# lpastura/kubernetes-1

Measured on AMD Instinct MI355X. Metric: pods scheduled/sec, higher is better.
Workload: dtype int64; 1 GPU; (b) 5000 nodes / 1913000 pods; nodes=5000, nodes_per_gpu=5000, pods=1913000, percentage_of_nodes_to_score=100, parallelism=1 GPU

## Files before the change

include/kgpu.h:

```cpp
#ifndef KGPU_H
#define KGPU_H

#include <stdint.h>

#ifdef __cplusplus
extern "C" {
#endif

#define KGPU_ABI_VERSION 3

#define KGPU_OK 0
#define KGPU_E_INVAL (-1)
#define KGPU_E_NOMEM (-2)
#define KGPU_E_DEVICE (-3)
#define KGPU_E_CAPACITY (-4)
#define KGPU_E_STATE (-5)
#define KGPU_E_UNSUPPORTED (-6)

#define KGPU_CODE_SUCCESS 0
#define KGPU_CODE_ERROR 1
#define KGPU_CODE_UNSCHEDULABLE 2
#define KGPU_CODE_UNRESOLVABLE 3

#define KGPU_F_NODE_UNSCHEDULABLE 0
// ... 392 lines not shown
#define KGPU_OPT_BATCH_GEO 11
#define KGPU_OPT_ARENA_BYTES 12
#define KGPU_OPT_TOPO_RESIDENT 13
#define KGPU_OPT_BATCH_HELPER 14
#define KGPU_OPT_TOPO_AHEAD 15
#define KGPU_OPT_TBATCH_GEO 16
#define KGPU_OPT_HOLD_GROUP 17
#define KGPU_OPT_TBATCH_WLAB 18
#define KGPU_OPT_RUN_ALL_FILTERS 20
#define KGPU_OPT_TBATCH_POLL_SLEEP 21
#define KGPU_OPT_ZEROCOPY_POOLS 23
#define KGPU_OPT_CUT_PERSISTENT 24
#define KGPU_OPT_CUT_TOPO_PERSISTENT 25
#define KGPU_OPT_NORM_PERSISTENT 26
#define KGPU_OPT_BATCH_EARLY_PUBLISH 27
int kgpu_set_option(kgpu_ctx* ctx, int32_t option, int64_t value);
int kgpu_debug_counters(const kgpu_ctx* ctx, int64_t* out, int32_t n);
int kgpu_geometry_for(int32_t kernel, int32_t n_nodes, int32_t max_groups, int32_t first, int32_t out[4]);
int kgpu_debug_geometry(const kgpu_ctx* ctx, int32_t out[6]);
int kgpu_debug_instantiation(const kgpu_ctx* ctx, int32_t out[4]);
int kgpu_debug_topo_resident(const kgpu_ctx* ctx, int64_t out[2]);
int kgpu_read_phase_trace(kgpu_ctx* ctx, int64_t* out, int32_t max_iters);

typedef struct kgpu_nominated {
  int32_t node;
  int32_t item;
} kgpu_nominated;
int kgpu_set_nominated(kgpu_ctx* ctx, const kgpu_nominated* noms, int32_t n, const kgpu_pod_query* pods,
                       const kgpu_pools* pools);

// ... 64 lines not shown
```

kubernetes-1_amd/csrc/kgpu_api.cpp:

```cpp
#include <hip/hip_runtime.h>
#include <rccl/rccl.h>
#include <dlfcn.h>
#include <execinfo.h>
#include <fcntl.h>
#include <signal.h>
#include <unistd.h>

#include <algorithm>
#include <array>
#include <chrono>
#include <atomic>
#include <exception>
#include <memory>
#include <new>
#include <iterator>
#include <cmath>
#include <cstdio>
#include <cstdlib>
#include <cstddef>
#include <cstring>
#include <deque>
#include <map>
#include <string>
#include <unordered_map>
// ... 149 lines not shown
    std::string key;
    DevBuf buf[2];
    size_t dirty[2] = {0, 0};
    int cur = 0;
  } tc;
  uint64_t tc_hits = 0, tc_misses = 0;
  bool htrace = false;
  static constexpr int kHt = 18;
  int64_t ht_last = 0, ht_cur[kHt] = {}, ht_n = 0;
  int ht_seen = 0;
  std::vector<std::array<int64_t, kHt>> ht_cycles;
  std::vector<std::array<int64_t, kHt>> ht_batches;
  bool tc_on = true;
  bool batch_helper = true;
  bool batch_early = true;
  bool topo_ahead = true;
  int tbatch_geo_first = 1;
  size_t ar_limit = 1 << 20;
  DevState ds_last{};
  const void* ds_ptr = nullptr;
  bool last_diag = false;
  std::vector<int64_t> trace_wg_host;
  int32_t trace_wg_groups = 0;
  std::vector<hipEvent_t> ev_pool;
  std::map<std::vector<int64_t>, int> class_ids, tclass_ids;
  std::vector<kgpu::ClassRec> classes;
  std::vector<kgpu::ClassItem> citems;
  std::vector<kgpu::TermClassRec> tclasses;
  std::vector<kgpu_req> creqs;
  std::vector<int32_t> cints;
// ... 109 lines not shown
      c->err = std::string(msg) + (what.empty() ? "" : ": " + what) +
               (invalidate ? " (device mirror invalidated: upload the snapshot again)" : "");
    } catch (...) {
      c->err.clear();
    }
  }
  return code;
}

void note_geometry(kgpu_ctx* c, int kernel, int geo, int groups, int per) {
  int threads = 0, rows = 0;
  kgpu::geometry_shape(kernel, geo, &threads, &rows);
  const int32_t v[6] = {kernel, geo, threads, rows, groups, per};
  std::copy(v, v + 6, c->last_geo);
}
void note_instantiation(kgpu_ctx* c, int row, bool xg, bool helper, int pods) {
  c->last_inst[0] = row;
  c->last_inst[1] = xg ? 1 : 0;
  c->last_inst[2] = helper ? 1 : 0;
  c->last_inst[3] += pods;
}
void reset_geometry(kgpu_ctx* c) {
  const int32_t v[6] = {0, -1, 0, 0, 0, 0};
  std::copy(v, v + 6, c->last_geo);
  const int32_t w[4] = {-1, 0, 0, 0};
  std::copy(w, w + 4, c->last_inst);
}

#define HIP_OK(c, x)                                                                           \
  do {                                                                                         \
    hipError_t e_ = (x);                                                                       \
    if (e_ != hipSuccess)                                                                      \
      return fail((c), KGPU_E_DEVICE, std::string(#x ": ") + hipGetErrorString(e_));           \
  } while (0)

// ... 1967 lines not shown
        ba.GT = groups;
      } else if (xg) {
        const size_t cells = (size_t)kgpu::kXgmiRing * (size_t)c->xg_GT;
        ba.gran = static_cast<uint64_t*>(c->xg_box.p);
        ba.feas = reinterpret_cast<int32_t*>(ba.gran + cells);
        ba.pgran = static_cast<uint64_t* const*>(c->xg_arr.p);
        ba.pfeas = reinterpret_cast<int32_t* const*>(static_cast<uint64_t* const*>(c->xg_arr.p) + c->xg_nranks);
        ba.nranks = c->xg_nranks;
        ba.rank = c->xg_rank;
        ba.GT = c->xg_GT;
        ba.R = kgpu::kXgmiRing;
        ba.xseq0 = c->xg_seq;
        c->xg_seq += cnt;
      } else {
        ba.dual = c->batch_early && kgpu::batch_helper_used(c->spec, kidx, false, c->batch_helper) ? 1 : 0;
        const size_t cells = (size_t)cnt * (size_t)groups * (ba.dual ? 2 : 1);
        const size_t gbytes = sizeof(uint64_t) * cells + sizeof(int32_t) * cells;
        if ((rc = ensure(c, c->gran, gbytes))) return rc;
        HIP_OK(c, hipMemsetAsync(c->gran.p, 0, sizeof(uint64_t) * cells, c->stream));
        ba.gran = static_cast<uint64_t*>(c->gran.p);
        ba.feas = reinterpret_cast<int32_t*>(ba.gran + cells);
        run_ptrs.push_back({ba.gran, ba.feas});
        void** slot = static_cast<void**>(c->batch_ptrs.p) + 2 * (run_ptrs.size() - 1);
        if ((rc = stage_h2d(c, slot, run_ptrs.back().data(), sizeof(void*) * 2))) return rc;
        ba.pgran = reinterpret_cast<uint64_t* const*>(slot);
        ba.pfeas = reinterpret_cast<int32_t* const*>(slot + 1);
        ba.nranks = 1;
        ba.rank = 0;
        ba.GT = groups;
        ba.R = 0;
      }
      ba.first = i;
      ba.count = cnt;
      ba.per = per;
      ba.assume = assume;
      ba.seq0 = first_seq + i;
      ba.abort = abort_word;
      ba.abort_at = c->abort_at >= i && c->abort_at < i + cnt ? c->abort_at - i : -1;
      ba.skip_release_at = c->skip_release_at >= i && c->skip_release_at < i + cnt ? c->skip_release_at - i : -1;
      ba.trace = nullptr;
      if (c->phase_trace) {
        if ((rc = ensure(c, c->trace, sizeof(int64_t) * 16 * (size_t)(cnt + 1)))) return rc;
        HIP_OK(c, hipMemsetAsync(c->trace.p, 0, sizeof(int64_t) * 16 * (size_t)(cnt + 1), c->stream));
        ba.trace = static_cast<int64_t*>(c->trace.p);
        c->trace_host.assign((size_t)(cnt + 1) * 16, 0);
      }
      if (c->timing) HIP_OK(c, hipEventRecord(get_event(c, ev), c->stream));
      const bool coop = c->coop || c->force_coop;
      ba.hold = coop ? -1 : c->hold_group;
      ++c->n_persist;
      c->n_coop += coop ? 1 : 0;
      ++c->state_launches;
      note_geometry(c, 1, kidx, groups, per);
      note_instantiation(c, kgpu::batch_row(c->spec), ba.R > 0,
                         !cut && kgpu::batch_helper_used(c->spec, kidx, ba.R > 0, c->batch_helper), cnt);
      if (cut) {
        c->n_cut_pods += cnt;
        cut_pods += cnt;
        if (kgpu::launch_cbatch(dst, ba, groups, kidx, c->spec, coop, c->stream))
          return fail(c, KGPU_E_DEVICE, "k_cbatch launch failed");
      } else if (kgpu::launch_batch(dst, ba, groups, kidx, c->spec, coop, c->batch_helper, c->stream))
        return fail(c, KGPU_E_DEVICE, "k_batch launch failed");
      if (c->timing) HIP_OK(c, hipEventRecord(get_event(c, ev + 1), c->stream));
      ev += 2;
      timed_passes += cnt;
      if (ba.trace)
        HIP_OK(c, hipMemcpyAsync(c->trace_host.data(), ba.trace, sizeof(int64_t) * 16 * (size_t)(cnt + 1),
                                 hipMemcpyDeviceToHost, c->stream));
      used_persistent = true;
    } else {
      while (j < n && (kidx < 0 || norm[(size_t)j]) && !topo[(size_t)j] && (nrm.empty() || !nrm[(size_t)j])) ++j;
      int prev = -1;
      bool resolved_in_final = false;
      for (int32_t k = i; k < j; ++k) {
        PodArgs a{};
        a.pod = k;
        a.prev = prev;
        a.prev_blocks = blocks;
        a.prev_parity = (k - 1) & 1;
        a.parity = k & 1;
        const bool one_launch = short_cycle && n == 1 && diag && !sharded && !cut &&
                                !(qs[k].flags & KGPU_Q_SCORE_ERROR) && !needs_norm(c, qs[k], pools);
// ... 850 lines not shown
  void* ptrs[2] = {gran, feas};
  std::memcpy(h + p_off, ptrs, sizeof(ptrs));
  std::memset(h + a_off, 0, 64);
  HIP_OK(c, hipMemcpyAsync(d, h, bytes, hipMemcpyHostToDevice, c->stream));
  c->tc.valid = false;
  kgpu::BatchArgs ba{};
  ba.gran = gran;
  ba.feas = feas;
  ba.pgran = reinterpret_cast<uint64_t* const*>(d + p_off);
  ba.pfeas = reinterpret_cast<int32_t* const*>(d + p_off + sizeof(void*));
  ba.nranks = 1;
  ba.rank = 0;
  ba.GT = groups;
  ba.R = 0;
  ba.dual = dual ? 1 : 0;
  ba.first = 0;
  ba.count = n;
  ba.per = per;
  ba.assume = 1;
  ba.seq0 = first_seq;
  ba.abort = reinterpret_cast<int32_t*>(d + a_off);
  ba.abort_at = -1;
  ba.skip_release_at = -1;
  ba.trace = nullptr;
  ba.res_out = static_cast<kgpu_result*>(ps.res_dev);
  ba.abort_out = reinterpret_cast<int32_t*>(static_cast<char*>(ps.res_dev) + sizeof(kgpu_result) * (size_t)n);
  kgpu_ctx::PipeSlot& po = c->pipe[s ^ 1];
  ba.zero_buf = static_cast<uint64_t*>(po.gran.p);
  ba.zero_n16 = po.gran.p ? (int64_t)(po.gran.bytes / 16) : 0;
  const bool coop = c->coop;
  ba.hold = -1;
  ++c->n_persist;
  c->n_coop += coop ? 1 : 0;
  *reinterpret_cast<int32_t*>(static_cast<char*>(ps.res) + sizeof(kgpu_result) * (size_t)n) = -1;
  const bool timed = stats != nullptr;
  if (timed) HIP_OK(c, hipEventRecord(ps.t0, c->stream));
  note_geometry(c, 1, kidx, groups, per);
  note_instantiation(c, kgpu::batch_row(c->spec), false, kgpu::batch_helper_used(c->spec, kidx, false, c->batch_helper), n);
  if (kgpu::launch_batch(reinterpret_cast<const DevState*>(d), ba, groups, kidx, c->spec, coop, c->batch_helper,
                         c->stream))
    return fail(c, KGPU_E_DEVICE, "k_batch launch failed");
  if (timed) HIP_OK(c, hipEventRecord(ps.t1, c->stream));
  HIP_OK(c, hipEventRecord(ps.done, c->stream));
  ps.gran_zeroed = 0;
  if (po.gran.p) po.gran_zeroed = po.gran.bytes;
  kgpu_ctx::PipeBatch b;
  b.slot = s;
  b.n = n;
  b.results = results;
  b.stats = stats;
  b.timed = timed;
  b.qs.assign(qs, qs + n);
  if (pools) {
// ... 166 lines not shown
  fail_point();
  std::unique_ptr<kgpu_ctx> holder(new kgpu_ctx());
  kgpu_ctx* c = holder.get();
  int ndev = 0;
  if (hipGetDeviceCount(&ndev) != hipSuccess || ndev <= 0) return KGPU_E_DEVICE;
  if (cfg->device < 0 || cfg->device >= ndev) return KGPU_E_INVAL;
  c->cfg = *cfg;
  c->device = cfg->device;
  if (hipSetDevice(c->device) != hipSuccess) return KGPU_E_DEVICE;
  {
    const char* e = std::getenv("KGPU_SYNC_SPIN");
    if (e && e[0] == '1') (void)hipSetDeviceFlags(hipDeviceScheduleSpin);
  }
  if (const char* e = std::getenv("KGPU_HOST_TRACE")) c->htrace = e[0] == '1';
  if (const char* e = std::getenv("KGPU_BATCH_EARLY_PUBLISH")) c->batch_early = e[0] != '0';
  if (hipStreamCreateWithFlags(&c->stream, hipStreamNonBlocking) != hipSuccess)
    return KGPU_E_DEVICE;
  hipDeviceProp_t prop;
  if (hipGetDeviceProperties(&prop, c->device) != hipSuccess) {
    (void)hipStreamDestroy(c->stream);
    return KGPU_E_DEVICE;
  }
  c->n_cus = prop.multiProcessorCount;
  DevState& st = c->st;
  st.n_filters = cfg->n_filters;
  std::memcpy(st.filters, cfg->filters, sizeof(st.filters));
  st.n_scores = cfg->n_scores;
  std::memcpy(st.scores, cfg->scores, sizeof(st.scores));
  for (int i = 0; i < KGPU_NUM_SCORES; ++i) st.weights[i] = std::max<int64_t>(cfg->score_weights[i], 1);
  for (int i = 0; i < KGPU_NUM_SCORES; ++i) st.w_of[i] = 0;
// ... 200 lines not shown
    return fail(c, KGPU_E_STATE, "pipelined batches in flight: complete them with kgpu_schedule_batch_wait first");
  if (!c) return KGPU_E_INVAL;
  if (option == KGPU_OPT_KERNEL_TIMING) c->timing = value != 0;
  else if (option == KGPU_OPT_PERSISTENT) c->persistent = value != 0;
  else if (option == KGPU_OPT_PERSIST_GROUPS) c->max_groups = (int)std::max<int64_t>(value, 0);
  else if (option == KGPU_OPT_PHASE_TRACE) {
    c->phase_trace = value != 0;
    c->phase_trace_mode = (int)std::min<int64_t>(std::max<int64_t>(value, 0), 3);
  }
  else if (option == KGPU_OPT_TOPO_FUSED) c->topo_fused = value != 0;
  else if (option == KGPU_OPT_TOPO_PERSISTENT) c->tfast = value != 0;
  else if (option == KGPU_OPT_COOPERATIVE) c->coop = value != 0;
  else if (option == KGPU_OPT_BATCH_GEO) c->batch_geo_first = (int)std::min<int64_t>(std::max<int64_t>(0, value), 6);
  else if (option == KGPU_OPT_BATCH_HELPER) c->batch_helper = value != 0;
  else if (option == KGPU_OPT_BATCH_EARLY_PUBLISH) c->batch_early = value != 0;
  else if (option == KGPU_OPT_TOPO_AHEAD) c->topo_ahead = value != 0;
  else if (option == KGPU_OPT_TBATCH_GEO) c->tbatch_geo_first = (int)std::min<int64_t>(std::max<int64_t>(value, 0), 4);
  else if (option == KGPU_OPT_TOPO_RESIDENT) {
    c->tc_on = value != 0;
    c->tc.valid = false;
  } else if (option == KGPU_OPT_ARENA_BYTES) c->ar_limit = (size_t)std::min<int64_t>(std::max<int64_t>(0, value), (int64_t)kArenaBytes);
  else if (option == KGPU_OPT_ABORT_AT) c->abort_at = value < 0 || value > INT32_MAX ? -1 : (int32_t)value;
  else if (option == KGPU_OPT_XGMI) c->xgmi = value != 0;
  else if (option == KGPU_OPT_TBATCH_WLAB) c->tbatch_wlab = value != 0;
  else if (option == KGPU_OPT_TBATCH_POLL_SLEEP) c->tbatch_sleep = value != 0;
  else if (option == KGPU_OPT_ZEROCOPY_POOLS) c->zc_pools = value != 0;
  else if (option == KGPU_OPT_RUN_ALL_FILTERS) c->run_all = value != 0;
  else if (option == KGPU_OPT_HOLD_GROUP) c->hold_group = value < 0 || value > INT32_MAX ? -1 : (int32_t)value;
  else if (option == KGPU_OPT_CUT_PERSISTENT) c->cut_persistent = value != 0;
  else if (option == KGPU_OPT_CUT_TOPO_PERSISTENT) c->cut_topo_persistent = value != 0;
// ... 1063 lines not shown
```

kubernetes-1_amd/csrc/kgpu_internal.h:

```cpp
#pragma once
#include <stdint.h>

#include "../../include/kgpu.h"

namespace kgpu {

constexpr int kBlock = 64;
constexpr int kMaxBlocks = 1024;
constexpr int kSelAnd = 0, kSelNothing = 1, kSelEmpty = 2;
constexpr uint64_t kMask40 = (1ull << 40) - 1;
constexpr int kMaxRanks = 64;

struct BlkStat {
  int32_t feasible;
  int32_t max_taint;
  int32_t max_na;
  int32_t pad;
};
struct BlkKey {
  uint64_t key;
  int32_t idx;
  int32_t feasible;
};

// ... 195 lines not shown
  int32_t hold;
  int32_t dual;
  kgpu_result* res_out;
  int32_t* abort_out;
  uint64_t* zero_buf;
  int64_t zero_n16;
  uint64_t* const* pgran;
  int32_t* const* pfeas;
  int32_t nranks, rank;
  int32_t GT;
  int32_t R;
  int64_t xseq0;
  uint64_t* cgran;
  uint64_t* cpos;
  int32_t cut_nofilt;
  int32_t pad_c;
};
constexpr int32_t kAbortDirty = 1, kAbortClean = 2;
constexpr int kXgmiRing = 4096;
constexpr int kXgmiMaxGT = 1024;

constexpr int kTMaxSoftWords = 8;
constexpr int kTMaxZones = 32;
constexpr int kTLdsBudget = 144 * 1024;
constexpr int kTCutBytes = 544;

struct THist {
  int32_t col_kind;
  int32_t col;
  int32_t key;
  int32_t sig;
// ... 160 lines not shown
int launch_vict_prep(const DevState* st, const PreemptArgs* a, void* stream);
int launch_victims(const DevState* st, const PreemptArgs* a, int N, void* stream);

int launch_eval(const DevState* st, const PodArgs& a, int blocks, int spec, void* stream);
int select_spec(const int32_t* filters, int nf, const int32_t* scores, int ns, bool def_res);
int launch_final(const DevState* st, const PodArgs& a, int blocks, int stat_blocks, void* stream);
int launch_cut(const DevState* st, const PodArgs& a, int blocks, int n_filters, void* stream);
int launch_resolve(const DevState* st, int N, const PodArgs& a, void* stream);
int eval_blocks(int N);
int launch_shard_pack(const DevState* st, int parity, int blocks, int what, void* stream);
int batch_geometry(int N, int max_groups, int* per, int* groups, int first = 0);
bool geometry_shape(int kernel, int geo, int* threads, int* rows);
int launch_batch(const DevState* st, const BatchArgs& a, int groups, int kidx, int spec, bool coop, bool helper,
                 void* stream);
int batch_row(int spec);
int launch_cbatch(const DevState* st, const BatchArgs& a, int groups, int kidx, int spec, bool coop, void* stream);
bool batch_helper_used(int spec, int geo, bool sharded, bool helper);
int launch_nbatch(const DevState* st, const BatchArgs& a, int groups, int kidx, int spec, bool coop, void* stream);
constexpr int kNormTaintBits = 20;
bool nbatch_row_ok(int spec);
int launch_topo(const DevState* st, PodArgs a, int blocks, int64_t min_values, int64_t next_scratch,
                bool fused, unsigned long long* bar, unsigned long long bar_base, int n_filters, void* stream,
                const PreemptArgs* nom = nullptr, int N = 0);
inline int topo_barriers(int64_t min_values) { return min_values > 0 ? 5 : 4; }
int launch_class_init(const DevState* st, int c0, int nc, int n_pods, void* stream);
int launch_debug_broken_linear(const kgpu_shape_point* pts, int n_pts, const int64_t* p, int64_t* out, int n,
                               void* stream);
int launch_debug_arith(int op, const int64_t* a, const int64_t* b, const int64_t* c, const int64_t* d, int64_t* out,
                       int32_t* flag, int n, void* stream);
int launch_topo_phase(const DevState* st, const PodArgs& a, int phase, int blocks, int64_t extra, void* stream);
// ... 45 lines not shown
```

kubernetes-1_amd/csrc/kgpu_kernels.hip:

```cpp
#include <hip/hip_runtime.h>

#include <algorithm>
#include <map>
#include <mutex>
#include <tuple>
#include <type_traits>

#include "kgpu_internal.h"

#if defined(__HIP_DEVICE_COMPILE__)
#define GAS __attribute__((address_space(1)))
#define CAS __attribute__((address_space(4)))
#else
#define GAS
#define CAS
#endif

namespace kgpu {

template <class T>
__device__ __forceinline__ GAS T* gp(T* p) {
  return (GAS T*)p;
}
template <class T>
__device__ __forceinline__ const CAS T* cp(const T* p) {
  return (const CAS T*)p;
}


constexpr uint32_t kRuntime = 0xFFFFFFFFu;
// ... 1165 lines not shown
    __builtin_amdgcn_s_sleep(1);
    if ((it & 63) == 0) {
      const uint64_t now = __builtin_amdgcn_s_memrealtime();
      if (it == 0) {
        t0 = now;
      } else if (now - t0 > 2 * kSpinTimeout) {
        __hip_atomic_fetch_or(abort_word, kAbortDirty, __ATOMIC_RELAXED, __HIP_MEMORY_SCOPE_AGENT);
        return;
      }
    }
  }
}
__device__ __forceinline__ void lds_wait(int* f, int v, int32_t* abort_word) { lds_wait_t<false>(f, v, abort_word); }
__device__ __forceinline__ void lds_wait_ge(int* f, int v, int32_t* abort_word) { lds_wait_t<true>(f, v, abort_word); }

__device__ __forceinline__ constexpr bool spare_slot(int j, int K, int tid, int B) {
  return j == K - 1 && tid == B - 1;
}

template <int K, int B>
__device__ __forceinline__ void wg_partials(BatchShared<B>& sh, int p, const uint64_t (&keys)[K], bool vb, int ob,
                                            int jb, int cand, Cand& ra, Cand& rb) {
  const int tid = threadIdx.x, lane = tid & 63, wave = tid >> 6;
  Cand a{0, -1, 0}, b{0, -1, 0};
  if (!vb) {
#pragma unroll
    for (int j = 0; j < K; ++j) {
      const uint64_t k = spare_slot(j, K, tid, B) ? 0 : keys[j];
      a.feas += __popcll(__ballot(k != 0));
      if (k > a.key) { a.key = k; a.idx = j * B + tid; }
// ... 198 lines not shown
  q.nz[0] = s.nz[0]; q.nz[1] = s.nz[1];
  q.score_req[0] = s.score_req[0]; q.score_req[1] = s.score_req[1];
  q.scalars = s.scalars;
  q.ports = s.ports;
  return q;
}
__device__ __forceinline__ kgpu_pod_query ring_uniform(kgpu_pod_query q) {
  q.flags = __builtin_amdgcn_readfirstlane(q.flags);
  q.scalars.begin = __builtin_amdgcn_readfirstlane(q.scalars.begin);
  q.scalars.count = __builtin_amdgcn_readfirstlane(q.scalars.count);
  q.ports.begin = __builtin_amdgcn_readfirstlane(q.ports.begin);
  q.ports.count = __builtin_amdgcn_readfirstlane(q.ports.count);
  return q;
}

template <uint32_t FM, uint32_t SM, int K, int B, bool XG, bool HB = false, bool TR = false, bool EP = false>
__global__ __launch_bounds__(B + 64 + (HB ? 2 * B : 0)) void k_batch(const DevState* __restrict__ stp, BatchArgs pa) {
  static_assert(!HB || (B == 64 && !XG &&
                       SM == ((1u << KGPU_S_BALANCED_ALLOCATION) | (1u << KGPU_S_LEAST_ALLOCATED) | kDefRes)),
                "the helper wave splits config (b)'s profile on the one-row-wave geometry");
  static_assert(HB || !TR, "only the helper-wave instantiation has a traced twin");
  static_assert(HB || !EP, "only the helper-wave instantiation publishes early");
  const DevState& st = *stp;
  constexpr int W = B / 64;
  const int tid = threadIdx.x, wave = tid >> 6, lane = tid & 63;
  const int G = gridDim.x, g = blockIdx.x;
  if (g == pa.hold) return;
  const int lo = g * pa.per;
  const int GT = pa.GT, gme = pa.rank * G + g;
  constexpr bool xg = XG;
  const uint64_t tmask = xg ? (0xFull << 60) : kGValid;
  __shared__ BatchShared<B> sh;
  __shared__ int64_t sh_hk[HB ? 2 * 2 * K * B : 1];
  __shared__ int sh_hready[2];
  __shared__ std::conditional_t<HB, kgpu_pod_query, NoQuery> sh_q[HB ? kQRing : 1];
  __shared__ uint64_t* sh_peer_g[XG ? kMaxRanks : 1];
  __shared__ int32_t* sh_peer_f[XG ? kMaxRanks : 1];
  if constexpr (XG) {
    if (wave == W && lane < pa.nranks) {
      sh_peer_g[lane] = pa.pgran[lane];
      sh_peer_f[lane] = pa.pfeas[lane];
    }
  }
  if (tid == 0) {
    sh.bready = 0;
    sh.cready = 0;
    sh_hready[0] = 0;
    sh_hready[1] = 0;
  }
  if constexpr (HB) {
    if (wave == W && lane < kQWords)
      for (int k = 0; k < 3 && k < pa.count; ++k)
        reinterpret_cast<qword_t*>(&sh_q[k])[lane] = ((const GAS qword_t*)(st.queries + pa.first + k))[lane];
  }
  __syncthreads();
  auto ring_row = [&](int k) -> size_t { return xg ? (size_t)((pa.xseq0 + k) % pa.R) : (size_t)k; };
  auto ring_tag = [&](int k) -> uint64_t {
    return xg ? (kGValid | ((uint64_t)(((pa.xseq0 + k) / pa.R) & 7) << 60)) : kGValid;
  };
  auto publish = [&](int i, uint64_t key, int feas) {
    const size_t roff = ring_row(i) * GT + gme;
    const uint64_t gtag = ring_tag(i);
    if constexpr (!XG) {
// ... 8 lines not shown
  };
  auto publish2 = [&](int i, uint64_t ka, uint64_t kb, int fa, int fb) {
    const size_t roff = (size_t)i * GT + gme;
    typedef uint32_t __attribute__((ext_vector_type(4))) u32x4;
    const uint64_t wa = kGValid | ka, wb = kGValid | kb;
    const u32x4 v = {(uint32_t)wa, (uint32_t)(wa >> 32), (uint32_t)wb, (uint32_t)(wb >> 32)};
    GAS uint64_t* gp2 = (GAS uint64_t*)(pa.gran + 2 * roff);
    asm volatile("global_store_dwordx4 %0, %1, off sc1\n\ts_nop 1" ::"v"(gp2), "v"(v) : "memory");
    reinterpret_cast<int2*>(pa.feas)[roff] = int2{fa, fb};
  };
  const bool tr = pa.trace && (g == 0 || g == G - 1);
  int64_t* trow = pa.trace ? pa.trace + (g == 0 ? 0 : 8) : nullptr;
  constexpr bool kStamps = !HB || TR;
#define KGPU_STAMP(i, k) \
  if (kStamps && tr && (tid == 0 || tid == B)) trow[(size_t)(i) * 16 + (k)] = (int64_t)__builtin_amdgcn_s_memrealtime()

  if constexpr (HB) {
    if (wave == W + 1 || wave == W + 2) {
      const int hw = wave - W - 1;
      HRow h[K];
#pragma unroll
      for (int j = 0; j < K; ++j) {
        const int n = lo + j * B + lane;
        h[j] = HRow{0, 0, 0, 0, 0.0, 0.0};
        if (!spare_slot(j, K, lane, B) && n < st.N) {
          h[j].ac = gp(st.alloc_cpu)[n];
          h[j].am = gp(st.alloc_mem)[n];
          h[j].zc = gp(st.nz_cpu)[n];
          h[j].zm = gp(st.nz_mem)[n];
          h[j].ic = (h[j].ac > 0 && h[j].ac < (1ll << 52)) ? 1.0 / (double)h[j].ac : 0.0;
// ... 24 lines not shown
                t.zm = lane64(h[j].zm, ob) + rqp.nz[1];
                t.ic = __builtin_bit_cast(double, lane64(__builtin_bit_cast(int64_t, h[j].ic), ob));
                t.im = __builtin_bit_cast(double, lane64(__builtin_bit_cast(int64_t, h[j].im), ob));
              }
            if (lane == B - 1) h[K - 1] = t;
          }
          kgpu_pod_query qh;
          qh.score_req[0] = rq.score_req[0];
          qh.score_req[1] = rq.score_req[1];
#pragma unroll
          for (int j = 0; j < K; ++j) {
            const bool spare = spare_slot(j, K, lane, B);
            const int n = spare ? lo + cand : lo + j * B + lane;
            NodeRes nr{};
            nr.ac = h[j].ac; nr.am = h[j].am; nr.zc = h[j].zc; nr.zm = h[j].zm; nr.ic = h[j].ic; nr.im = h[j].im;
            sh_hk[((hw * 2 + p) * K + j) * B + lane] =
                hw == 0 ? least_score<true>(st, qh, nr, n) * wl : balanced_score(qh, nr) * wbal;
          }
          if (lane == 0) lds_release(&sh_hready[hw], i + 1);
        }
        __syncthreads();
        int wg = -1;
        if (have_prev) {
          if (sh.rabort[(i - 1) & 1]) break;
          wg = sh.rwg[(i - 1) & 1];
        }
        const bool won = have_prev && wg == gme;
        if (won && pa.assume && lane == ob) {
#pragma unroll
          for (int j = 0; j < K; ++j)
            if (j == jb) {
              h[j].zc += rqp.nz[0];
              h[j].zm += rqp.nz[1];
            }
// ... 153 lines not shown
        }
        assume_regs(qp, t);
        if (tid == B - 1) r[KR - 1] = t;
      }
      if constexpr (HB) {
        uint32_t fs[K];
        uint64_t rkj[K];
#pragma unroll
        for (int j = 0; j < K; ++j) {
          const bool spare = spare_slot(j, K, tid, B);
          const int n = spare ? lo + cand : lo + j * B + tid;
          fs[j] = (spare ? fast_b : n < st.N) ? run_filters<FM>(st, q, r[j], n) : 1u;
          rkj[j] = rank40(tk, (uint64_t)(st.node_base + n), st.tie_mode);
        }
        if (q.scalars.count | q.ports.count) vm_drain();
        lds_wait_ge(&sh_hready[0], i + 1, pa.abort);
        lds_wait_ge(&sh_hready[1], i + 1, pa.abort);
#pragma unroll
        for (int j = 0; j < K; ++j) {
          const int64_t tot = sh_hk[((0 * 2 + p) * K + j) * B + tid] + sh_hk[((1 * 2 + p) * K + j) * B + tid];
          keys[j] = fs[j] ? 0 : (((uint64_t)(tot + 1) << 40) | rkj[j]);
        }
      } else {
#pragma unroll
        for (int j = 0; j < K; ++j) {
          const bool spare = spare_slot(j, K, tid, B);
          const int n = spare ? lo + cand : lo + j * B + tid;
          if constexpr (kStream) {
            const bool live = spare ? fast_b : n < st.N;
            NodeRes rj = r[0];
            if (!spare && live) rj = load_row<kRecip>(st, n);
            keys[j] = live ? node_key<FM, SM>(st, q, rj, n, tk) : 0;
          } else {
            keys[j] = (spare ? fast_b : n < st.N) ? node_key<FM, SM>(st, q, r[j], n, tk) : 0;
          }
        }
// ... 83 lines not shown
#pragma unroll
        for (int j = 0; j < K; ++j)
          if (j == cand / B) {
            if constexpr (kStream) sh.brow[p] = load_row<kRecip>(st, lo + cand);
            else sh.brow[p] = r[j];
          }
        if (i != pa.skip_release_at) lds_release(&sh.bready, i + 1);
      }
    }
    staged = have_cur && !slow && cand >= 0;
    qp = q;
    q = qn;
    KGPU_STAMP(i, 4);
  }
#undef KGPU_STAMP
}

__global__ __launch_bounds__(256) void k_batch_fixup(const DevState* __restrict__ stp, BatchArgs pa, int G) {
  const DevState& st = *stp;
  const int lane = threadIdx.x & 63;
  const int i = blockIdx.x * 4 + (threadIdx.x >> 6);
  for (int64_t z = (int64_t)blockIdx.x * blockDim.x + threadIdx.x; z < pa.zero_n16; z += (int64_t)gridDim.x * blockDim.x) {
    uint4* zp = reinterpret_cast<uint4*>(pa.zero_buf) + z;
    *zp = uint4{0, 0, 0, 0};
  }
  if (pa.abort_out && blockIdx.x == 0 && threadIdx.x == 0)
    __hip_atomic_store(pa.abort_out, load_sc1(pa.abort), __ATOMIC_RELAXED, __HIP_MEMORY_SCOPE_SYSTEM);
  if (i >= pa.count) return;
  const size_t row = pa.R > 0 ? (size_t)((pa.xseq0 + i) % pa.R) : (size_t)i;
  int f = 0;
// ... 2772 lines not shown
template <uint32_t FM, uint32_t SM>
struct BatchRow {
  using Fn = void (*)(const DevState*, BatchArgs);
  static constexpr Fn fn[kNumGeo] = {k_batch<FM, SM, 1, 64, false>,  k_batch<FM, SM, 1, 128, false>,
                                     k_batch<FM, SM, 1, 192, false>, k_batch<FM, SM, 1, 448, false>,
                                     k_batch<FM, SM, 1, 960, false>, k_batch<FM, SM, 4, 512, false>,
                                     k_batch<FM, SM, 8, 512, false>};
  static constexpr Fn xfn[kNumGeo] = {k_batch<FM, SM, 1, 64, true>,  k_batch<FM, SM, 1, 128, true>,
                                      k_batch<FM, SM, 1, 192, true>, k_batch<FM, SM, 1, 448, true>,
                                      k_batch<FM, SM, 1, 960, true>, k_batch<FM, SM, 4, 512, true>,
                                      k_batch<FM, SM, 8, 512, true>};
};
using BatchFn = void (*)(const DevState*, BatchArgs);
template <uint32_t FM, uint32_t SM, bool E>
struct HelperFn {
  static constexpr BatchFn fn = nullptr, traced = nullptr, early = nullptr, early_traced = nullptr;
};
template <uint32_t FM, uint32_t SM>
struct HelperFn<FM, SM, true> {
  static constexpr BatchFn fn = k_batch<FM, SM, 1, 64, false, true>;
  static constexpr BatchFn traced = k_batch<FM, SM, 1, 64, false, true, true>;
  static constexpr BatchFn early = k_batch<FM, SM, 1, 64, false, true, false, true>;
  static constexpr BatchFn early_traced = k_batch<FM, SM, 1, 64, false, true, true, true>;
};
static const BatchFn kBatchHelper[] = {
    nullptr,
    HelperFn<kFitFM, kFitSM, true>::fn,
    nullptr,
    nullptr,
};
static const BatchFn kBatchHelperTraced[] = {
    nullptr,
    HelperFn<kFitFM, kFitSM, true>::traced,
    nullptr,
    nullptr,
};
static const BatchFn kBatchHelperEarly[] = {
    nullptr,
    HelperFn<kFitFM, kFitSM, true>::early,
    nullptr,
    nullptr,
};
static const BatchFn kBatchHelperEarlyTraced[] = {
    nullptr,
    HelperFn<kFitFM, kFitSM, true>::early_traced,
    nullptr,
    nullptr,
};
static const BatchFn* const kBatch[] = {
    BatchRow<kRuntime, kRuntime>::fn,
    BatchRow<kFitFM, kFitSM>::fn,
    BatchRow<kDefaultFM, kDefaultSM>::fn,
    BatchRow<kDefaultFM, kAutoscalerSM>::fn,
};
static_assert(sizeof(kBatch) / sizeof(kBatch[0]) == kNumSpecs, "one k_batch row per profile instantiation");
static const BatchFn* const kBatchX[] = {
    BatchRow<kRuntime, kRuntime>::xfn,
    BatchRow<kFitFM, kFitSM>::xfn,
    BatchRow<kDefaultFM, kDefaultSM>::xfn,
    BatchRow<kDefaultFM, kAutoscalerSM>::xfn,
};

int batch_geometry(int N, int max_groups, int* per, int* groups, int first) {
// ... 26 lines not shown
int batch_row(int spec) { return spec < 0 || spec >= kNumSpecs ? 0 : spec; }

bool batch_helper_used(int spec, int geo, bool sharded, bool helper) {
  return helper && !sharded && geo == 0 && kBatchHelper[batch_row(spec)] != nullptr;
}

int launch_batch(const DevState* st, const BatchArgs& a, int groups, int geo, int spec, bool coop, bool helper,
                 void* stream) {
  spec = batch_row(spec);
  if (geo < 0 || geo >= kNumGeo) return -1;
  const int x = a.R > 0 ? 1 : 0;
  const bool hb = batch_helper_used(spec, geo, x != 0, helper);
  const bool traced = hb && a.trace != nullptr;
  const bool early = a.dual != 0;
  if (early && !hb) return -1;
  const BatchFn fn = hb ? (early ? (traced ? kBatchHelperEarlyTraced : kBatchHelperEarly)
                                 : (traced ? kBatchHelperTraced : kBatchHelper))[spec]
                        : (x ? kBatchX : kBatch)[spec][geo];
  const int threads = kGeo[geo].B + 64 + (hb ? 2 * kGeo[geo].B : 0);
  static bool attr_set[6][kNumSpecs][kNumGeo] = {};
  const int ai = hb ? (traced ? 3 : 2) + (early ? 2 : 0) : x;
  if (!attr_set[ai][spec][geo]) {
    if (hipFuncSetAttribute(reinterpret_cast<const void*>(fn), hipFuncAttributeMaxDynamicSharedMemorySize,
                            kBatchLdsPad) != hipSuccess)
      return -1;
    attr_set[ai][spec][geo] = true;
  }
  BatchArgs arg = a;
  const DevState* sp = st;
  void* args[] = {(void*)&sp, (void*)&arg};
  if (!coop && grid_fits(reinterpret_cast<const void*>(fn), threads, (size_t)kBatchLdsPad, groups)) {
    hipLaunchKernelGGL(fn, dim3(groups), dim3(threads), (unsigned)kBatchLdsPad, (hipStream_t)stream, sp, arg);
    if (hipGetLastError() != hipSuccess) return -1;
  } else {
    arg.hold = -1;
    if (hipLaunchCooperativeKernel(reinterpret_cast<const void*>(fn), dim3(groups), dim3(threads), args,
// ... 687 lines not shown
```

kubernetes-1_amd/kgpu/abi.py:

```python
import ctypes as C

import numpy as np

ABI_VERSION = 3
OK, E_INVAL, E_NOMEM, E_DEVICE, E_CAPACITY, E_STATE, E_UNSUPPORTED = 0, -1, -2, -3, -4, -5, -6
ERRNAMES = {0: "OK", -1: "KGPU_E_INVAL", -2: "KGPU_E_NOMEM", -3: "KGPU_E_DEVICE", -4: "KGPU_E_CAPACITY",
            -5: "KGPU_E_STATE", -6: "KGPU_E_UNSUPPORTED"}

OPT_KERNEL_TIMING, OPT_PERSISTENT, OPT_PERSIST_GROUPS, OPT_PHASE_TRACE, OPT_TOPO_FUSED = 1, 2, 3, 4, 5
OPT_TOPO_PERSISTENT = 6
OPT_ABORT_AT = 7
OPT_XGMI = 8
OPT_SKIP_RELEASE_AT = 9
OPT_COOPERATIVE = 10
OPT_BATCH_GEO = 11
OPT_ARENA_BYTES = 12
OPT_TOPO_RESIDENT = 13
OPT_BATCH_HELPER = 14
OPT_TOPO_AHEAD = 15
OPT_TBATCH_GEO = 16
OPT_HOLD_GROUP = 17
OPT_TBATCH_WLAB = 18
OPT_RUN_ALL_FILTERS = 20
OPT_TBATCH_POLL_SLEEP = 21
OPT_ZEROCOPY_POOLS = 23
OPT_CUT_PERSISTENT = 24
OPT_CUT_TOPO_PERSISTENT = 25
OPT_NORM_PERSISTENT = 26
OPT_BATCH_EARLY_PUBLISH = 27
CODE_SUCCESS, CODE_ERROR, CODE_UNSCHEDULABLE, CODE_UNRESOLVABLE = 0, 1, 2, 3
STATUS_NOT_EVALUATED = 0xFF

F_NODE_UNSCHEDULABLE, F_FIT, F_NODE_NAME, F_NODE_PORTS, F_NODE_AFFINITY, F_TAINT, F_PTS, F_IPA = range(8)
NUM_FILTERS = 8
FILTER_IDS = {"NodeUnschedulable": 0, "NodeResourcesFit": 1, "NodeName": 2, "NodePorts": 3, "NodeAffinity": 4,
              "TaintToleration": 5, "PodTopologySpread": 6, "InterPodAffinity": 7}
FILTER_NAMES = {v: k for k, v in FILTER_IDS.items()}

(S_BALANCED, S_IMAGE, S_IPA, S_LEAST, S_NODE_AFFINITY, S_NPAP, S_PTS, S_DPTS, S_TAINT, S_MOST, S_RTCR,
 S_LIMITS) = range(12)
NUM_SCORES = 12
SCORE_IDS = {"NodeResourcesBalancedAllocation": 0, "ImageLocality": 1, "InterPodAffinity": 2,
             "NodeResourcesLeastAllocated": 3, "NodeAffinity": 4, "NodePreferAvoidPods": 5,
             "PodTopologySpread": 6, "DefaultPodTopologySpread": 7, "TaintToleration": 8,
# ... 144 lines not shown
```

kubernetes-1_amd/kgpu/native.py:

```python
import ctypes as C
import os

import numpy as np

from . import abi

_HERE = os.path.dirname(os.path.abspath(__file__))
LIB_PATH = os.environ.get("KGPU_LIB_PATH") or os.path.join(_HERE, "libkgpu.so")
_lib = None

EXPORTS = ["kgpu_abi_version", "kgpu_struct_sizes", "kgpu_create", "kgpu_destroy", "kgpu_last_error",
           "kgpu_upload_snapshot", "kgpu_generation", "kgpu_schedule_one", "kgpu_schedule_batch",
           "kgpu_get_filter", "kgpu_get_filter_all", "kgpu_get_scores", "kgpu_forget_pod", "kgpu_read_nodes", "kgpu_set_option",
           "kgpu_read_phase_trace", "kgpu_comm_unique_id", "kgpu_comm_init", "kgpu_apply_delta",
           "kgpu_set_nominated", "kgpu_select_victims", "kgpu_xgmi_handle", "kgpu_xgmi_init", "kgpu_xgmi_active",
           "kgpu_comm_info",
           "kgpu_debug_fail_alloc", "kgpu_debug_pts_state", "kgpu_debug_ipa_state", "kgpu_debug_broken_linear",
           "kgpu_debug_wg_trace", "kgpu_debug_topo_resident",
           "kgpu_next_slot", "kgpu_adopt_pod", "kgpu_prepare_pods", "kgpu_filter_reasons", "kgpu_debug_counters",
           "kgpu_schedule_batch_submit", "kgpu_schedule_batch_wait", "kgpu_pipelined",
           "kgpu_geometry_for", "kgpu_debug_geometry", "kgpu_debug_instantiation", "kgpu_debug_arith"]


class KgpuError(RuntimeError):
# ... 279 lines not shown

    def topo_resident(self):
        out = np.zeros(2, np.int64)
        self._check(lib().kgpu_debug_topo_resident(self.h, out.ctypes.data))
        return int(out[0]), int(out[1])

    def geometry(self):
        out = np.zeros(6, np.int32)
        self._check(lib().kgpu_debug_geometry(self.h, out.ctypes.data))
        return {"kernel": _GEO_KERNELS[int(out[0])], "index": int(out[1]), "threads": int(out[2]),
                "rows_per_lane": int(out[3]), "groups": int(out[4]), "per": int(out[5])}

    def instantiation(self):
        out = np.zeros(4, np.int32)
        self._check(lib().kgpu_debug_instantiation(self.h, out.ctypes.data))
        return {"row": int(out[0]), "sharded": bool(out[1]), "helper": bool(out[2]), "persistent_pods": int(out[3])}

    def counters(self):
        out = np.zeros(8, np.int64)
        n = lib().kgpu_debug_counters(self.h, out.ctypes.data, len(out))
        if n < 0:
            self._check(n)
        return dict(zip(["coop_retries", "persistent_launches", "coop_launches", "class_inits", "pod_table_full_uploads",
                         "cut_persistent_pods", "cut_topo_persistent_pods", "norm_persistent_pods"],
                        [int(x) for x in out[:n]]))

    def broken_linear(self, points, utilizations):
        pts = (abi.ShapePoint * len(points))()
        for i, (u, sc) in enumerate(points):
            pts[i].utilization, pts[i].score = int(u), int(sc)
        p = np.ascontiguousarray(utilizations, np.int64)
# ... 70 lines not shown
```

Measured before the change: 795,900 pods/s.

## Replace helper-wave ready flags with per-slot tagged score hand-offs in LDS

In the helper-wave batch kernel, the two helper waves now write each weighted score together with a pod-sequence tag as one 64-bit LDS word. The main wave polls these tagged pairs with a single 128-bit LDS read instead of waiting on two shared ready counters. This removes the whole-wave release/acquire on sh_hready, so the main wave can consume each slot as soon as that slot is written. Scores that do not fit in 32 bits get tag 0, and the path is only enabled when the score weights keep them in range. It adds a new kernel instantiation, an option and an env switch, and it spins per slot, which risks more LDS polling traffic.

```diff
diff --git a/include/kgpu.h b/include/kgpu.h
--- a/include/kgpu.h
+++ b/include/kgpu.h
@@ -430,6 +430,7 @@
 #define KGPU_OPT_CUT_TOPO_PERSISTENT 25
 #define KGPU_OPT_NORM_PERSISTENT 26
 #define KGPU_OPT_BATCH_EARLY_PUBLISH 27
+#define KGPU_OPT_BATCH_HANDOFF 28
 int kgpu_set_option(kgpu_ctx* ctx, int32_t option, int64_t value);
 int kgpu_debug_counters(const kgpu_ctx* ctx, int64_t* out, int32_t n);
 int kgpu_geometry_for(int32_t kernel, int32_t n_nodes, int32_t max_groups, int32_t first, int32_t out[4]);
diff --git a/kubernetes-1_amd/csrc/kgpu_api.cpp b/kubernetes-1_amd/csrc/kgpu_api.cpp
--- a/kubernetes-1_amd/csrc/kgpu_api.cpp
+++ b/kubernetes-1_amd/csrc/kgpu_api.cpp
@@ -187,6 +187,7 @@
   bool tc_on = true;
   bool batch_helper = true;
   bool batch_early = true;
+  bool batch_handoff = true;
   bool topo_ahead = true;
   int tbatch_geo_first = 1;
   size_t ar_limit = 1 << 20;
@@ -326,11 +327,14 @@
   const int32_t v[6] = {kernel, geo, threads, rows, groups, per};
   std::copy(v, v + 6, c->last_geo);
 }
-void note_instantiation(kgpu_ctx* c, int row, bool xg, bool helper, int pods) {
+void note_instantiation(kgpu_ctx* c, int row, bool xg, bool helper, int pods, bool handoff = false) {
   c->last_inst[0] = row;
   c->last_inst[1] = xg ? 1 : 0;
-  c->last_inst[2] = helper ? 1 : 0;
+  c->last_inst[2] = (helper ? 1 : 0) | (helper && handoff ? 2 : 0);
   c->last_inst[3] += pods;
+}
+bool handoff_wanted(const kgpu_ctx* c) {
+  return c->batch_handoff && kgpu::batch_handoff_fits(c->st.w_of[KGPU_S_LEAST_ALLOCATED], c->st.w_of[KGPU_S_BALANCED_ALLOCATION]);
 }
 void reset_geometry(kgpu_ctx* c) {
   const int32_t v[6] = {0, -1, 0, 0, 0, 0};
@@ -2328,6 +2332,7 @@
         c->xg_seq += cnt;
       } else {
         ba.dual = c->batch_early && kgpu::batch_helper_used(c->spec, kidx, false, c->batch_helper) ? 1 : 0;
+        ba.handoff = ba.dual && handoff_wanted(c) ? 1 : 0;
         const size_t cells = (size_t)cnt * (size_t)groups * (ba.dual ? 2 : 1);
         const size_t gbytes = sizeof(uint64_t) * cells + sizeof(int32_t) * cells;
         if ((rc = ensure(c, c->gran, gbytes))) return rc;
@@ -2354,10 +2359,10 @@
       ba.skip_release_at = c->skip_release_at >= i && c->skip_release_at < i + cnt ? c->skip_release_at - i : -1;
       ba.trace = nullptr;
       if (c->phase_trace) {
-        if ((rc = ensure(c, c->trace, sizeof(int64_t) * 16 * (size_t)(cnt + 1)))) return rc;
-        HIP_OK(c, hipMemsetAsync(c->trace.p, 0, sizeof(int64_t) * 16 * (size_t)(cnt + 1), c->stream));
+        if ((rc = ensure(c, c->trace, sizeof(int64_t) * 16 * 2 * (size_t)(cnt + 1)))) return rc;
+        HIP_OK(c, hipMemsetAsync(c->trace.p, 0, sizeof(int64_t) * 16 * 2 * (size_t)(cnt + 1), c->stream));
         ba.trace = static_cast<int64_t*>(c->trace.p);
-        c->trace_host.assign((size_t)(cnt + 1) * 16, 0);
+        c->trace_host.assign((size_t)(cnt + 1) * 16 * 2, 0);
       }
       if (c->timing) HIP_OK(c, hipEventRecord(get_event(c, ev), c->stream));
       const bool coop = c->coop || c->force_coop;
@@ -2367,7 +2372,8 @@
       ++c->state_launches;
       note_geometry(c, 1, kidx, groups, per);
       note_instantiation(c, kgpu::batch_row(c->spec), ba.R > 0,
-                         !cut && kgpu::batch_helper_used(c->spec, kidx, ba.R > 0, c->batch_helper), cnt);
+                         !cut && kgpu::batch_helper_used(c->spec, kidx, ba.R > 0, c->batch_helper), cnt,
+                         !cut && ba.handoff != 0);
       if (cut) {
         c->n_cut_pods += cnt;
         cut_pods += cnt;
@@ -2379,7 +2385,7 @@
       ev += 2;
       timed_passes += cnt;
       if (ba.trace)
-        HIP_OK(c, hipMemcpyAsync(c->trace_host.data(), ba.trace, sizeof(int64_t) * 16 * (size_t)(cnt + 1),
+        HIP_OK(c, hipMemcpyAsync(c->trace_host.data(), ba.trace, sizeof(int64_t) * 16 * 2 * (size_t)(cnt + 1),
                                  hipMemcpyDeviceToHost, c->stream));
       used_persistent = true;
     } else {
@@ -3260,6 +3266,7 @@
   ba.GT = groups;
   ba.R = 0;
   ba.dual = dual ? 1 : 0;
+  ba.handoff = dual && handoff_wanted(c) ? 1 : 0;
   ba.first = 0;
   ba.count = n;
   ba.per = per;
@@ -3282,7 +3289,8 @@
   const bool timed = stats != nullptr;
   if (timed) HIP_OK(c, hipEventRecord(ps.t0, c->stream));
   note_geometry(c, 1, kidx, groups, per);
-  note_instantiation(c, kgpu::batch_row(c->spec), false, kgpu::batch_helper_used(c->spec, kidx, false, c->batch_helper), n);
+  note_instantiation(c, kgpu::batch_row(c->spec), false, kgpu::batch_helper_used(c->spec, kidx, false, c->batch_helper), n,
+                     ba.handoff != 0);
   if (kgpu::launch_batch(reinterpret_cast<const DevState*>(d), ba, groups, kidx, c->spec, coop, c->batch_helper,
                          c->stream))
     return fail(c, KGPU_E_DEVICE, "k_batch launch failed");
@@ -3479,6 +3487,7 @@
   }
   if (const char* e = std::getenv("KGPU_HOST_TRACE")) c->htrace = e[0] == '1';
   if (const char* e = std::getenv("KGPU_BATCH_EARLY_PUBLISH")) c->batch_early = e[0] != '0';
+  if (const char* e = std::getenv("KGPU_BATCH_HANDOFF")) c->batch_handoff = e[0] != '0';
   if (hipStreamCreateWithFlags(&c->stream, hipStreamNonBlocking) != hipSuccess)
     return KGPU_E_DEVICE;
   hipDeviceProp_t prop;
@@ -3709,6 +3718,7 @@
   else if (option == KGPU_OPT_BATCH_GEO) c->batch_geo_first = (int)std::min<int64_t>(std::max<int64_t>(0, value), 6);
   else if (option == KGPU_OPT_BATCH_HELPER) c->batch_helper = value != 0;
   else if (option == KGPU_OPT_BATCH_EARLY_PUBLISH) c->batch_early = value != 0;
+  else if (option == KGPU_OPT_BATCH_HANDOFF) c->batch_handoff = value != 0;
   else if (option == KGPU_OPT_TOPO_AHEAD) c->topo_ahead = value != 0;
   else if (option == KGPU_OPT_TBATCH_GEO) c->tbatch_geo_first = (int)std::min<int64_t>(std::max<int64_t>(value, 0), 4);
   else if (option == KGPU_OPT_TOPO_RESIDENT) {
diff --git a/kubernetes-1_amd/csrc/kgpu_internal.h b/kubernetes-1_amd/csrc/kgpu_internal.h
--- a/kubernetes-1_amd/csrc/kgpu_internal.h
+++ b/kubernetes-1_amd/csrc/kgpu_internal.h
@@ -233,7 +233,7 @@
   uint64_t* cgran;
   uint64_t* cpos;
   int32_t cut_nofilt;
-  int32_t pad_c;
+  int32_t handoff;
 };
 constexpr int32_t kAbortDirty = 1, kAbortClean = 2;
 constexpr int kXgmiRing = 4096;
@@ -424,6 +424,10 @@
 int launch_batch(const DevState* st, const BatchArgs& a, int groups, int kidx, int spec, bool coop, bool helper,
                  void* stream);
 int batch_row(int spec);
+inline bool batch_handoff_fits(int64_t w_least, int64_t w_balanced) {
+  return w_least >= 0 && w_balanced >= 0 && w_least <= (int64_t)(0xFFFFFFFFull / 100) &&
+         w_balanced <= (int64_t)(0xFFFFFFFFull / 100);
+}
 int launch_cbatch(const DevState* st, const BatchArgs& a, int groups, int kidx, int spec, bool coop, void* stream);
 bool batch_helper_used(int spec, int geo, bool sharded, bool helper);
 int launch_nbatch(const DevState* st, const BatchArgs& a, int groups, int kidx, int spec, bool coop, void* stream);
diff --git a/kubernetes-1_amd/csrc/kgpu_kernels.hip b/kubernetes-1_amd/csrc/kgpu_kernels.hip
--- a/kubernetes-1_amd/csrc/kgpu_kernels.hip
+++ b/kubernetes-1_amd/csrc/kgpu_kernels.hip
@@ -11,9 +11,11 @@
 #if defined(__HIP_DEVICE_COMPILE__)
 #define GAS __attribute__((address_space(1)))
 #define CAS __attribute__((address_space(4)))
+#define LAS __attribute__((address_space(3)))
 #else
 #define GAS
 #define CAS
+#define LAS
 #endif
 
 namespace kgpu {
@@ -1209,6 +1211,30 @@
 __device__ __forceinline__ void lds_wait(int* f, int v, int32_t* abort_word) { lds_wait_t<false>(f, v, abort_word); }
 __device__ __forceinline__ void lds_wait_ge(int* f, int v, int32_t* abort_word) { lds_wait_t<true>(f, v, abort_word); }
 
+__device__ __forceinline__ void lds_wait_tagged(const int64_t* pair, uint32_t tag, int32_t* abort_word, uint32_t& a,
+                                                uint32_t& b) {
+  typedef uint32_t __attribute__((ext_vector_type(4))) u32x4;
+  const uint32_t addr = (uint32_t)(uintptr_t)(LAS const int64_t*)pair;
+  uint64_t t0 = 0;
+  for (int it = 0;; ++it) {
+    u32x4 v;
+    asm volatile("ds_read_b128 %0, %1\n\ts_waitcnt lgkmcnt(0)" : "=v"(v) : "v"(addr) : "memory");
+    a = v.x;
+    b = v.z;
+    if (__builtin_amdgcn_ballot_w64(v.y != tag || v.w != tag) == 0) return;
+    __builtin_amdgcn_s_sleep(1);
+    if ((it & 63) == 0) {
+      const uint64_t now = __builtin_amdgcn_s_memrealtime();
+      if (it == 0) {
+        t0 = now;
+      } else if (now - t0 > 2 * kSpinTimeout) {
+        __hip_atomic_fetch_or(abort_word, kAbortDirty, __ATOMIC_RELAXED, __HIP_MEMORY_SCOPE_AGENT);
+        return;
+      }
+    }
+  }
+}
+
 __device__ __forceinline__ constexpr bool spare_slot(int j, int K, int tid, int B) {
   return j == K - 1 && tid == B - 1;
 }
@@ -1437,13 +1463,15 @@
   return q;
 }
 
-template <uint32_t FM, uint32_t SM, int K, int B, bool XG, bool HB = false, bool TR = false, bool EP = false>
+template <uint32_t FM, uint32_t SM, int K, int B, bool XG, bool HB = false, bool TR = false, bool EP = false,
+          bool HO = false>
 __global__ __launch_bounds__(B + 64 + (HB ? 2 * B : 0)) void k_batch(const DevState* __restrict__ stp, BatchArgs pa) {
   static_assert(!HB || (B == 64 && !XG &&
                        SM == ((1u << KGPU_S_BALANCED_ALLOCATION) | (1u << KGPU_S_LEAST_ALLOCATED) | kDefRes)),
                 "the helper wave splits config (b)'s profile on the one-row-wave geometry");
   static_assert(HB || !TR, "only the helper-wave instantiation has a traced twin");
   static_assert(HB || !EP, "only the helper-wave instantiation publishes early");
+  static_assert((HB && EP) || !HO, "tagged hand-offs: the early-publish helper-wave instantiation only");
   const DevState& st = *stp;
   constexpr int W = B / 64;
   const int tid = threadIdx.x, wave = tid >> 6, lane = tid & 63;
@@ -1454,7 +1482,7 @@
   constexpr bool xg = XG;
   const uint64_t tmask = xg ? (0xFull << 60) : kGValid;
   __shared__ BatchShared<B> sh;
-  __shared__ int64_t sh_hk[HB ? 2 * 2 * K * B : 1];
+  __shared__ __attribute__((aligned(HO ? 16 : 8))) int64_t sh_hk[HB ? 2 * 2 * K * B : 1];
   __shared__ int sh_hready[2];
   __shared__ std::conditional_t<HB, kgpu_pod_query, NoQuery> sh_q[HB ? kQRing : 1];
   __shared__ uint64_t* sh_peer_g[XG ? kMaxRanks : 1];
@@ -1470,6 +1498,9 @@
     sh.cready = 0;
     sh_hready[0] = 0;
     sh_hready[1] = 0;
+  }
+  if constexpr (HO) {
+    for (int k = tid; k < 2 * 2 * K * B; k += B + 64 + 2 * B) sh_hk[k] = 0;
   }
   if constexpr (HB) {
     if (wave == W && lane < kQWords)
@@ -1508,6 +1539,9 @@
   constexpr bool kStamps = !HB || TR;
 #define KGPU_STAMP(i, k) \
   if (kStamps && tr && (tid == 0 || tid == B)) trow[(size_t)(i) * 16 + (k)] = (int64_t)__builtin_amdgcn_s_memrealtime()
+#define KGPU_HSTAMP(i, k, who)                  \
+  if (HB && TR && tr && tid == (who))           \
+  trow[((size_t)pa.count + 1 + (i)) * 16 + (k)] = (int64_t)__builtin_amdgcn_s_memrealtime()
 
   if constexpr (HB) {
     if (wave == W + 1 || wave == W + 2) {
@@ -1562,10 +1596,19 @@
             const int n = spare ? lo + cand : lo + j * B + lane;
             NodeRes nr{};
             nr.ac = h[j].ac; nr.am = h[j].am; nr.zc = h[j].zc; nr.zm = h[j].zm; nr.ic = h[j].ic; nr.im = h[j].im;
-            sh_hk[((hw * 2 + p) * K + j) * B + lane] =
-                hw == 0 ? least_score<true>(st, qh, nr, n) * wl : balanced_score(qh, nr) * wbal;
+            const int64_t ws = hw == 0 ? least_score<true>(st, qh, nr, n) * wl : balanced_score(qh, nr) * wbal;
+            if constexpr (HO) {
+              const uint64_t tag = ((uint64_t)ws >> 32) == 0 ? (uint64_t)(uint32_t)(i + 1) : 0;
+              __hip_atomic_store(reinterpret_cast<uint64_t*>(&sh_hk[(((p * K + j) * B + lane) << 1) + hw]),
+                                 (tag << 32) | (uint32_t)ws, __ATOMIC_RELAXED, __HIP_MEMORY_SCOPE_WORKGROUP);
+            } else {
+              sh_hk[((hw * 2 + p) * K + j) * B + lane] = ws;
+            }
           }
-          if (lane == 0) lds_release(&sh_hready[hw], i + 1);
+          if constexpr (!HO) {
+            if (lane == 0) lds_release(&sh_hready[hw], i + 1);
+          }
+          KGPU_HSTAMP(i, 2, B + 64 + B);
         }
         __syncthreads();
         int wg = -1;
@@ -1749,12 +1792,25 @@
           rkj[j] = rank40(tk, (uint64_t)(st.node_base + n), st.tie_mode);
         }
         if (q.scalars.count | q.ports.count) vm_drain();
-        lds_wait_ge(&sh_hready[0], i + 1, pa.abort);
-        lds_wait_ge(&sh_hready[1], i + 1, pa.abort);
-#pragma unroll
-        for (int j = 0; j < K; ++j) {
-          const int64_t tot = sh_hk[((0 * 2 + p) * K + j) * B + tid] + sh_hk[((1 * 2 + p) * K + j) * B + tid];
-          keys[j] = fs[j] ? 0 : (((uint64_t)(tot + 1) << 40) | rkj[j]);
+        KGPU_HSTAMP(i, 0, 0);
+        if constexpr (HO) {
+#pragma unroll
+          for (int j = 0; j < K; ++j) {
+            uint32_t sl, sb;
+            lds_wait_tagged(&sh_hk[((p * K + j) * B + tid) << 1], (uint32_t)(i + 1), pa.abort, sl, sb);
+            if (j == K - 1) KGPU_HSTAMP(i, 1, 0);
+            const int64_t tot = (int64_t)sl + (int64_t)sb;
+            keys[j] = fs[j] ? 0 : (((uint64_t)(tot + 1) << 40) | rkj[j]);
+          }
+        } else {
+          lds_wait_ge(&sh_hready[0], i + 1, pa.abort);
+          lds_wait_ge(&sh_hready[1], i + 1, pa.abort);
+          KGPU_HSTAMP(i, 1, 0);
+#pragma unroll
+          for (int j = 0; j < K; ++j) {
+            const int64_t tot = sh_hk[((0 * 2 + p) * K + j) * B + tid] + sh_hk[((1 * 2 + p) * K + j) * B + tid];
+            keys[j] = fs[j] ? 0 : (((uint64_t)(tot + 1) << 40) | rkj[j]);
+          }
         }
       } else {
 #pragma unroll
@@ -1868,6 +1924,7 @@
     KGPU_STAMP(i, 4);
   }
 #undef KGPU_STAMP
+#undef KGPU_HSTAMP
 }
 
 __global__ __launch_bounds__(256) void k_batch_fixup(const DevState* __restrict__ stp, BatchArgs pa, int G) {
@@ -4670,7 +4727,8 @@
 using BatchFn = void (*)(const DevState*, BatchArgs);
 template <uint32_t FM, uint32_t SM, bool E>
 struct HelperFn {
-  static constexpr BatchFn fn = nullptr, traced = nullptr, early = nullptr, early_traced = nullptr;
+  static constexpr BatchFn fn = nullptr, traced = nullptr, early = nullptr, early_traced = nullptr, handoff = nullptr,
+                           handoff_traced = nullptr;
 };
 template <uint32_t FM, uint32_t SM>
 struct HelperFn<FM, SM, true> {
@@ -4678,6 +4736,8 @@
   static constexpr BatchFn traced = k_batch<FM, SM, 1, 64, false, true, true>;
   static constexpr BatchFn early = k_batch<FM, SM, 1, 64, false, true, false, true>;
   static constexpr BatchFn early_traced = k_batch<FM, SM, 1, 64, false, true, true, true>;
+  static constexpr BatchFn handoff = k_batch<FM, SM, 1, 64, false, true, false, true, true>;
+  static constexpr BatchFn handoff_traced = k_batch<FM, SM, 1, 64, false, true, true, true, true>;
 };
 static const BatchFn kBatchHelper[] = {
     nullptr,
@@ -4703,6 +4763,18 @@
     nullptr,
     nullptr,
 };
+static const BatchFn kBatchHelperHandoff[] = {
+    nullptr,
+    HelperFn<kFitFM, kFitSM, true>::handoff,
+    nullptr,
+    nullptr,
+};
+static const BatchFn kBatchHelperHandoffTraced[] = {
+    nullptr,
+    HelperFn<kFitFM, kFitSM, true>::handoff_traced,
+    nullptr,
+    nullptr,
+};
 static const BatchFn* const kBatch[] = {
     BatchRow<kRuntime, kRuntime>::fn,
     BatchRow<kFitFM, kFitSM>::fn,
@@ -4759,12 +4831,15 @@
   const bool traced = hb && a.trace != nullptr;
   const bool early = a.dual != 0;
   if (early && !hb) return -1;
-  const BatchFn fn = hb ? (early ? (traced ? kBatchHelperEarlyTraced : kBatchHelperEarly)
-                                 : (traced ? kBatchHelperTraced : kBatchHelper))[spec]
+  const bool handoff = a.handoff != 0;
+  if (handoff && !early) return -1;
+  const BatchFn fn = hb ? (handoff ? (traced ? kBatchHelperHandoffTraced : kBatchHelperHandoff)
+                           : early ? (traced ? kBatchHelperEarlyTraced : kBatchHelperEarly)
+                                   : (traced ? kBatchHelperTraced : kBatchHelper))[spec]
                         : (x ? kBatchX : kBatch)[spec][geo];
   const int threads = kGeo[geo].B + 64 + (hb ? 2 * kGeo[geo].B : 0);
-  static bool attr_set[6][kNumSpecs][kNumGeo] = {};
-  const int ai = hb ? (traced ? 3 : 2) + (early ? 2 : 0) : x;
+  static bool attr_set[8][kNumSpecs][kNumGeo] = {};
+  const int ai = hb ? (traced ? 3 : 2) + (early ? 2 : 0) + (handoff ? 2 : 0) : x;
   if (!attr_set[ai][spec][geo]) {
     if (hipFuncSetAttribute(reinterpret_cast<const void*>(fn), hipFuncAttributeMaxDynamicSharedMemorySize,
                             kBatchLdsPad) != hipSuccess)
diff --git a/kubernetes-1_amd/kgpu/abi.py b/kubernetes-1_amd/kgpu/abi.py
--- a/kubernetes-1_amd/kgpu/abi.py
+++ b/kubernetes-1_amd/kgpu/abi.py
@@ -28,6 +28,7 @@
 OPT_CUT_TOPO_PERSISTENT = 25
 OPT_NORM_PERSISTENT = 26
 OPT_BATCH_EARLY_PUBLISH = 27
+OPT_BATCH_HANDOFF = 28
 CODE_SUCCESS, CODE_ERROR, CODE_UNSCHEDULABLE, CODE_UNRESOLVABLE = 0, 1, 2, 3
 STATUS_NOT_EVALUATED = 0xFF
 
diff --git a/kubernetes-1_amd/kgpu/native.py b/kubernetes-1_amd/kgpu/native.py
--- a/kubernetes-1_amd/kgpu/native.py
+++ b/kubernetes-1_amd/kgpu/native.py
@@ -317,7 +317,8 @@
     def instantiation(self):
         out = np.zeros(4, np.int32)
         self._check(lib().kgpu_debug_instantiation(self.h, out.ctypes.data))
-        return {"row": int(out[0]), "sharded": bool(out[1]), "helper": bool(out[2]), "persistent_pods": int(out[3])}
+        return {"row": int(out[0]), "sharded": bool(out[1]), "helper": bool(out[2] & 1), "handoff": bool(out[2] & 2),
+                "persistent_pods": int(out[3])}
 
     def counters(self):
         out = np.zeros(8, np.int64)
```

After: 782,500 pods/s. -1.7%, worse.
